# lRomul/sensorium

Hardware: AMD Instinct MI355X
Metric: training clips/sec/GPU (DwiseNeuro fwd+bwd, B=32 T=32 36x64) at 1/2/4/8 GPUs (higher is better)
Workload: dtype bf16

## Files before the change

sensorium_amd/csrc/dwn_api.hip:

```cpp
#include "dwn_internal.h"
#include "dwn_kernels.h"
#include <string.h>
#include <math.h>

static thread_local char g_err[512] = "";
#ifndef DWN_EVAL_CHAIN
#define DWN_EVAL_CHAIN 1
#endif

extern "C" size_t dwn_dw_spatial_rc_blob_bytes(int E, int Cin);
extern "C" int dwn_dw_spatial_rc_supported(int dtype, int Cin, int E, int ks, int stride, int Hin, int Win);
extern "C" int dwn_dw_spatial_rc_prep(const float* w_pw, const float* w_dws, const float* bn1_coef, int E, int Cin, void* blob,
                                      int device, void* stream);
extern "C" int dwn_dw_spatial_fwd_rc(const dwn_dw_spatial_rc_fwd_args* a, int device, void* stream);
bool dw_spatial_bwd_rc_supported(const DwSpatialBwd& a, int dtype);
bool dw_spatial_fwd_rc_walk_supported(const DwSpatialFwd& a, int dtype);

int dwn_set_error(int code, const char* msg) {
    snprintf(g_err, sizeof(g_err), "dwn error %d: %s", code, msg ? msg : "");
    return code;
}

#define TRY(x) do { int rc__ = (x); if (rc__ != 0) return rc__; } while (0)

// ... 110 lines not shown
}

int bn_finalize(const double* stats, int stat_c, double count, const dwn_bn& bn, int C, int training, float momentum,
                float eps, hipStream_t s) {
    if (training) return k_bn_finalize_train(fin_job(stats, stat_c, count, bn, C), BnFinJob{}, momentum, eps, s);
    return k_bn_finalize_eval(bn.gamma, bn.beta, bn.running_mean, bn.running_var, eps, bn.coef, C, s);
}

GemmNN nn_base(const LoadDesc& a, int a_kind, const void* b, i64 ldb, void* c, i64 ldc, int M, int N, int K, int groups) {
    GemmNN g; memset(&g, 0, sizeof(g));
    g.a = a; g.a_kind = a_kind; g.b = b; g.ldb = ldb; g.c = c; g.ldc = ldc; g.M = M; g.N = N; g.K = K;
    g.groups = groups; g.epi = EPI_STORE;
    return g;
}
GemmTN tn_base(const LoadDesc& p, int pk, const LoadDesc& q, int qk, int M, int R, int Cc, float* dw, i64 lddw, int groups) {
    GemmTN g; memset(&g, 0, sizeof(g));
    g.p = p; g.p_kind = pk; g.q = q; g.q_kind = qk; g.M = M; g.R = R; g.Cc = Cc; g.dw = dw; g.lddw = lddw;
    g.groups = groups; g.nsplit = 0;
    return g;
}

struct BlockWs {
    void *wpw, *wpwl;
    float *wdws, *wdwt;
    double *st1, *st2, *st3, *st4, *stsc;
    long long* pooled;
    float *abc1, *abc2, *abc3, *abc4, *abcsc, *ident3;
    float *dgp, *dhp, *dps;
    void* bp; float* r3; float* gacc;
    float* tacc;
    void* wgated;
    void* rcblob;
    double* gram;
    float* pb;
    char* zero_beg; char* zero_end;
    size_t bytes;
};
#ifndef PWL_GATED_MIN_ROWS
#define PWL_GATED_MIN_ROWS 8192
#endif
static bool pwl_gated_weights(const dwn_block_args& a) {
    const int bk = a.dtype == DWN_BF16 ? 64 : 32;
    return ((a.T * a.Hout * a.Wout) % 128) == 0 && a.Cmid > bk && (a.dtype != DWN_BF16 || a.T * a.Hout * a.Wout >= PWL_GATED_MIN_ROWS);
}
static bool pwl_bwd_per_sample(const dwn_block_args& a) {
#ifdef DWN_DETERMINISTIC
    return true;
#endif
    if (a.pwl_bwd == 2) return false;
    if (a.pwl_bwd == 1) return true;
    const double pb = 4.0 * a.B * a.Cout * a.Cmid * sizeof(float);
    const double pass = (double)a.B * a.T * a.Hout * a.Wout * a.Cmid * tsize(a.dtype);
    return pb <= pass;
}
static bool block_y1_free(const dwn_block_args& a) {
    if (!a.training || a.dtype != DWN_BF16 || a.y1_mode == 1) return false;
    DwSpatialFwd f; memset(&f, 0, sizeof(f));
    f.planes = a.B * a.T; f.Hin = a.Hin; f.Win = a.Win; f.Hout = a.Hout; f.Wout = a.Wout; f.C = a.Cmid; f.stride = a.stride; f.ks = a.ks;
    f.in.ld = a.Cmid; f.a0_ld = a.Cin; f.Cin = a.Cin;
    if (!dw_spatial_fwd_rc_walk_supported(f, a.dtype)) return false;
    DwSpatialBwd d; memset(&d, 0, sizeof(d));
    d.planes = a.B * a.T; d.Hin = a.Hin; d.Win = a.Win; d.Hout = a.Hout; d.Wout = a.Wout; d.C = a.Cmid; d.stride = a.stride; d.ks = a.ks;
    d.dy.ld = a.Cmid; d.y1.ld = a.Cmid; d.a0_ld = a.Cin; d.Cin = a.Cin;
    if (!dw_spatial_bwd_rc_supported(d, a.dtype)) return false;
    return a.y1_mode == 2 || a.Cin == 64;
}
static bool block_fwd_rc(const dwn_block_args& a) {
    return !a.training && dwn_dw_spatial_rc_supported(a.dtype, a.Cin, a.Cmid, a.ks, a.stride, a.Hin, a.Win) != 0;
}
static size_t pw_fold_floats(int Cin) { return (size_t)Cin * Cin + Cin; }
BlockWs carve_block(const dwn_block_args& a, int backward, void* base, size_t cap) {
    BlockWs w; memset(&w, 0, sizeof(w));
    Carver c(base, cap);
    const size_t ts = tsize(a.dtype);
    w.wpw = c.take<char>((size_t)a.Cmid * a.Cin * ts);
    w.wpwl = c.take<char>((size_t)a.Cout * a.Cmid * ts);
    w.wdws = c.take<float>((size_t)a.ks * a.ks * a.Cmid);
    w.wdwt = c.take<float>((size_t)a.kt * a.Cmid);
    if (!backward && pwl_gated_weights(a)) w.wgated = c.take<char>((size_t)a.B * a.Cout * a.Cmid * ts);
    if (!backward && block_fwd_rc(a)) w.rcblob = c.take<char>(dwn_dw_spatial_rc_blob_bytes(a.Cmid, a.Cin));
    c.take<char>(0);
    size_t z0 = (c.off + 255) & ~(size_t)255;
    w.st1 = c.take<double>(nstat(a.Cmid));
    w.st2 = c.take<double>(nstat(a.Cmid));
    w.st3 = c.take<double>(nstat(a.Cmid));
    w.st4 = c.take<double>(nstat(a.Cout));
    w.stsc = c.take<double>(nstat(backward ? a.Cout : a.Cin));
    w.pooled = c.take<long long>((size_t)a.B * a.Cmid);
    if (!backward && block_y1_free(a)) w.gram = c.take<double>((size_t)(a.Cin + 8) * a.Cin);
    size_t z1 = c.off;
    if (backward) {
        w.abc1 = c.take<float>(3 * (size_t)a.Cmid);
        w.abc2 = c.take<float>(3 * (size_t)a.Cmid);
        w.abc3 = c.take<float>(3 * (size_t)a.Cmid);
        w.abc4 = c.take<float>(3 * (size_t)a.Cout);
        w.abcsc = c.take<float>(3 * (size_t)a.Cout);
        w.ident3 = c.take<float>(3 * (size_t)a.Cmid);
        w.dgp = c.take<float>((size_t)a.B * a.Cmid);
        w.dhp = c.take<float>((size_t)a.B * a.se_r);
        w.dps = c.take<float>((size_t)a.B * a.Cmid);
        w.bp = c.take<char>((size_t)a.Cin * (a.Cmid + a.Cin) * ts);
        w.gacc = c.take<float>(pw_fold_floats(a.Cin));
        w.r3 = w.gacc + (size_t)a.Cin * a.Cin;
        w.tacc = c.take<float>(pw_wgrad_tacc_floats(a.Cmid, a.Cin));
        if (pwl_bwd_per_sample(a)) w.pb = c.take<float>((size_t)a.B * a.Cout * a.Cmid);
    }
    w.bytes = c.off + 256;
    if (base) { w.zero_beg = (char*)base + z0; w.zero_end = (char*)base + z1; }
    return w;
}

static inline int f32_split_of(int policy, bool eval_forward) {
    return policy == DWN_F32_SPLIT3 ? 1 : policy == DWN_F32_NATIVE ? 0 : (eval_forward ? 1 : 0);
}

ResGeom geom_of(const dwn_block_args& a) {
    ResGeom gm;
    gm.BT = a.B * a.T; gm.T = a.T; gm.Hin = a.Hin; gm.Win = a.Win; gm.Hout = a.Hout; gm.Wout = a.Wout;
    gm.Cin = a.Cin; gm.Cout = a.Cout; gm.hsrc = a.hsrc; gm.wsrc = a.wsrc; gm.hinv = a.hinv; gm.winv = a.winv;
    return gm;
}

int check_block(const dwn_block_args& a) {
// ... 72 lines not shown
int dwn_dw_spatial_fwd_rc_supported(const dwn_dw_spatial_fwd_args* a, int dtype) { return dw_spatial_fwd_rc_walk_supported(*a, dtype) ? 1 : 0; }
int dwn_dw_temporal_fwd(const dwn_dw_temporal_fwd_args* a, int dtype, int device, void* stream) {
    ENTER(device);
    if (a->kt != 3 && a->kt != 5) return dwn_set_error(-4, "dw_temporal: only temporal_kernel 3 or 5 is built");
    return launch_dw_temporal_fwd(*a, dtype, (hipStream_t)stream);
}
int dwn_dw_temporal_bwd(const dwn_dw_temporal_bwd_args* a, int dtype, int device, void* stream) {
    ENTER(device);
    if (a->kt != 3 && a->kt != 5) return dwn_set_error(-4, "dw_temporal: only temporal_kernel 3 or 5 is built");
    return launch_dw_temporal_bwd(*a, dtype, (hipStream_t)stream);
}
int dwn_dw_temporal_wide_fwd(const dwn_dw_temporal_fwd_args* a, int dtype, int device, void* stream) {
    g_err[0] = 0;
    if (int rc = dw_temporal_wide_check(a->kt, a->C, LD_PLAIN)) return rc;
    ENTER(device);
    return launch_dw_temporal_wide_fwd(*a, dtype, (hipStream_t)stream);
}
int dwn_dw_temporal_wide_bwd(const dwn_dw_temporal_bwd_args* a, int dtype, int device, void* stream) {
    g_err[0] = 0;
    if (int rc = dw_temporal_wide_check(a->kt, a->C, a->dy_kind)) return rc;
    ENTER(device);
    return launch_dw_temporal_wide_bwd(*a, dtype, (hipStream_t)stream);
}
int dwn_bn_finalize(const double* stats, int stat_c, double count, const dwn_bn* bn, int C, int training,
                    float momentum, float eps, int device, void* stream) {
    ENTER(device);
    return bn_finalize(stats, stat_c, count, *bn, C, training, momentum, eps, (hipStream_t)stream);
}
int dwn_bn_bwd_finalize(const double* stats, double count, const dwn_bn* bn, float* abc, int C, int device,
                        void* stream) {
    ENTER(device);
    return k_bn_bwd_finalize(bwd_job(stats, count, *bn, abc, C, false), BnBwdJob{}, (hipStream_t)stream);
}
size_t dwn_conv_pw_bn_stats_workspace_bytes(int Cin) { return (size_t)(Cin + 8) * Cin * sizeof(double) + 256; }
int dwn_conv_pw_bn_stats(const void* a0, long long a0_ld, long long M, const float* w_pw, int E, int Cin, const dwn_bn* bn,
                         float momentum, float eps, double* sc_stats, void* ws, size_t ws_bytes, int dtype, int device, void* stream) {
    ENTER(device);
    hipStream_t s = (hipStream_t)stream;
    if (!a0 || !w_pw || !bn || !bn->coef || !ws) return dwn_set_error(-1, "conv_pw_bn_stats: null pointer");
    if (Cin % 8 || E <= 0 || M <= 0 || M >= (1ll << 31)) return dwn_set_error(-2, "conv_pw_bn_stats: Cin % 8 == 0, 0 < M < 2^31");
    if (ws_bytes < dwn_conv_pw_bn_stats_workspace_bytes(Cin)) return dwn_set_error(-6, "conv_pw_bn_stats: workspace too small");
    double* gram = reinterpret_cast<double*>(((size_t)ws + 255) & ~(size_t)255);
    TRY(k_zero(gram, (size_t)(Cin + 8) * Cin * sizeof(double), s));
    LoadDesc cat = ld_plain(a0, a0_ld);
    cat.cat_c1 = Cin; cat.cat_c2 = 0;
    GemmTN g = tn_base(cat, LD_CAT1, ld_plain(a0, a0_ld), LD_PLAIN, (int)M, Cin + 8, Cin, reinterpret_cast<float*>(gram), Cin, 1);
    g.dw_f64 = 1;
    TRY(launch_gemm_tn(g, dtype, s));
    return k_bn1_gram_finalize(gram, w_pw, E, Cin, (double)M, bn->gamma, bn->beta, bn->running_mean, bn->running_var,
                               bn->num_batches_tracked, momentum, eps, bn->coef, sc_stats, dtype, s);
}
int dwn_pack_weight(const float* src, void* dst, int groups, int R, int C, int transpose, int Rd, int Cd, int dtype,
                    int device, void* stream) {
    ENTER(device);
    return k_pack_weight(src, dst, groups, R, C, transpose, Rd, Cd, dtype, (hipStream_t)stream);
}

size_t dwn_stem_workspace_bytes(const dwn_stem_args* a) {
    return ((size_t)DWN_NREP * stem_moment_count() * sizeof(double) + 256 +
            (size_t)DWN_NREP * a->C0 * stem_acc_stride() * sizeof(double) + 1024);
}
int dwn_stem_forward(const dwn_stem_args* a, int device, void* stream) {
    ENTER(device);
    hipStream_t s = (hipStream_t)stream;
    if (a->C0 % 8) return dwn_set_error(-2, "stem: C0 must be a multiple of 8");
    if (a->pe_t && (i64)a->T * a->H * a->W != a->S) return dwn_set_error(-2, "stem: T*H*W != S");
    Carver c(a->ws, a->ws_bytes);
    double* mom = c.take<double>((size_t)DWN_NREP * stem_moment_count());
    if (!c.ok()) return dwn_set_error(-6, "stem: workspace too small");
    const i64 M = (i64)a->B * a->S;
    if (a->training == DWN_BN_TRAIN) {
        if (!a->xmom) return dwn_set_error(-1, "stem_forward: xmom buffer required in training mode");
        TRY(k_zero(mom, (size_t)DWN_NREP * stem_moment_count() * sizeof(double), s));
        TRY(k_stem_xmom(a->x, a->B, a->Cin, a->S, mom, s));
        TRY(k_stem_bn_finalize(mom, (double)M, a->w, a->bn.gamma, a->bn.beta, a->bn.running_mean, a->bn.running_var,
// ... 91 lines not shown
            ok = ok && pa.bneval(a.bn1, a.Cmid, a.eps) && pa.bneval(a.bn2, a.Cmid, a.eps) && pa.bneval(a.bn3, a.Cmid, a.eps);
            ok = ok && pa.bneval(a.bn4, a.Cout, a.eps) && pa.bneval(a.bnsc, a.Cout, a.eps);
        }
        if (!ok) return dwn_set_error(-2, "block_forward: workspace arena must be 16-byte aligned");
        TRY(k_prep(pa, dt, s));
    }

    const void* a0 = a.x;
    if (!a.x_has_pe) {
        if (!a.a0) return dwn_set_error(-2, "block_forward: a0 buffer required when x_has_pe == 0");
        TRY(k_ew_apply(ld_pe(a.x, a.Cin, a.pe_t, a.pe_h, a.pe_w, a.T, a.Hin, a.Win), LD_PE, a.a0, a.Cin, Min, a.Cin, dt, s));
        a0 = a.a0;
    }
    LoadDesc xin = ld_plain(a0, a.Cin);
    const bool identity_sc = a.stride == 1 && a.Hin == a.Hout && a.Win == a.Wout;
    const bool y1_free = tr && block_y1_free(a);
    bool eval_chain = false;
    if (DWN_EVAL_CHAIN && !tr && dt == DWN_BF16) {
        DwSpatialFwd f; memset(&f, 0, sizeof(f));
        f.planes = a.B * a.T; f.Hin = a.Hin; f.Win = a.Win; f.Hout = a.Hout; f.Wout = a.Wout; f.C = a.Cmid; f.stride = a.stride; f.ks = a.ks;
        f.in.ld = a.Cmid; f.a0_ld = a.Cin; f.Cin = a.Cin;
        eval_chain = dw_spatial_fwd_rc_walk_supported(f, dt);
    }
    if (eval_chain) {
        DwSpatialFwd d; memset(&d, 0, sizeof(d));
        d.in = ld_bnact(nullptr, a.Cmid, a.bn1.coef, a.Cmid, 1, nullptr, 0, 1);
        d.a0 = a0; d.a0_ld = a.Cin; d.w1 = w.wpw; d.Cin = a.Cin;
        d.w = w.wdws; d.out = a.y2; d.planes = a.B * a.T; d.Hin = a.Hin; d.Win = a.Win; d.Hout = a.Hout;
        d.Wout = a.Wout; d.C = a.Cmid; d.stride = a.stride; d.ks = a.ks; d.stats = nullptr;
        PROF(DWN_FAM_DWS_FWD, launch_dw_spatial_fwd(d, dt, s));
    } else if (y1_free) {
        LoadDesc cat = ld_plain(a0, a.Cin);
        cat.cat_c1 = a.Cin; cat.cat_c2 = 0;
        if (bs) {
        GemmTN g = tn_base(cat, LD_CAT1, ld_plain(a0, a.Cin), LD_PLAIN, (int)Min, a.Cin + 8, a.Cin, reinterpret_cast<float*>(w.gram), a.Cin, 1);
        g.dw_f64 = 1;
        PROF(DWN_FAM_PW_FWD, launch_gemm_tn(g, dt, s));
        PROF(DWN_FAM_PW_FWD, k_bn1_gram_finalize(w.gram, a.w_pw, a.Cmid, a.Cin, (double)Min, a.bn1.gamma, a.bn1.beta, a.bn1.running_mean,
                                                 a.bn1.running_var, a.bn1.num_batches_tracked, a.momentum, a.eps, a.bn1.coef,
                                                 identity_sc ? w.stsc : nullptr, dt, s));
        }
        DwSpatialFwd d; memset(&d, 0, sizeof(d));
        d.in = ld_bnact(nullptr, a.Cmid, a.bn1.coef, a.Cmid, 1, nullptr, 0, 1);
        d.a0 = a0; d.a0_ld = a.Cin; d.w1 = w.wpw; d.Cin = a.Cin;
        d.w = w.wdws; d.out = a.y2; d.planes = a.B * a.T; d.Hin = a.Hin; d.Win = a.Win; d.Hout = a.Hout;
        d.Wout = a.Wout; d.C = a.Cmid; d.stride = a.stride; d.ks = a.ks; d.stats = w.st2;
        PROF(DWN_FAM_DWS_FWD, launch_dw_spatial_fwd(d, dt, s));
    } else if (block_fwd_rc(a)) {
        TRY(dwn_dw_spatial_rc_prep(a.w_pw, w.wdws, a.bn1.coef, a.Cmid, a.Cin, w.rcblob, device, stream));
        dwn_dw_spatial_rc_fwd_args r; memset(&r, 0, sizeof(r));
        r.a0 = a0; r.a0_ld = a.Cin; r.blob = w.rcblob; r.out = a.y2; r.planes = a.B * a.T; r.Hin = a.Hin; r.Win = a.Win;
        r.Hout = a.Hout; r.Wout = a.Wout; r.Cin = a.Cin; r.E = a.Cmid; r.stride = a.stride; r.stats = nullptr;
        r.rows_band = 0; r.round_y1 = 1;
        PROF(DWN_FAM_DWS_FWD, dwn_dw_spatial_fwd_rc(&r, device, stream));
    } else {
    {
        GemmNN g = nn_base(xin, LD_PLAIN, w.wpw, a.Cin, a.y1, a.Cmid, (int)Min, a.Cmid, a.Cin, 1);
        g.f32_split = f32_split_of(a.f32_products, !tr);
        g.stats = tr ? w.st1 : nullptr; g.stat_nchan = a.Cmid;
        PROF(DWN_FAM_PW_FWD, launch_gemm_nn(g, dt, s));
    }
    if (bs) TRY(bn_finalize(w.st1, a.Cmid, (double)Min, a.bn1, a.Cmid, 1, a.momentum, a.eps, s));
    {
        DwSpatialFwd d; memset(&d, 0, sizeof(d));
        d.in = ld_bnact(a.y1, a.Cmid, a.bn1.coef, a.Cmid, 1, nullptr, 0, 1);
        d.w = w.wdws; d.out = a.y2; d.planes = a.B * a.T; d.Hin = a.Hin; d.Win = a.Win; d.Hout = a.Hout;
        d.Wout = a.Wout; d.C = a.Cmid; d.stride = a.stride; d.ks = a.ks; d.stats = tr ? w.st2 : nullptr;
// ... 584 lines not shown
```

sensorium_amd/csrc/dwn_elementwise.hip:

```cpp
#include "dwn_internal.h"
#include "dwn_kernels.h"
#include "dwn_launch.h"

#define NCV 8
#define DISPATCH_T(dtype, CALL_BF, CALL_F) do { if ((dtype) == DWN_BF16) { CALL_BF; } else { CALL_F; } } while (0)

#define SLICE_SETUP(Cval)                                   \
    constexpr int KC = TT<T>::KC;                           \
    const int tid = threadIdx.x;                            \
    const int cv = tid % NCV, pl = tid / NCV;               \
    const int c0 = blockIdx.y * NCV * KC;                   \
    const int chan = c0 + cv * KC;                          \
    const bool chan_ok = chan < (Cval);                     \
    (void)pl; (void)chan_ok;

template <int KC>
__device__ __forceinline__ void slice_stats_flush(float* lstat, const float* s0, const float* s1, int cv,
                                                 int c0, int C, double* stats, int rep) {
    static_assert(NCV == 8, "wave pre-reduction below assumes 8 channel vectors per slice");
    const int tid = threadIdx.x;
    DET_WAVES_BEGIN
#pragma unroll
    for (int i = 0; i < KC; ++i) {
        float a = s0[i], b = s1[i];
// ... 168 lines not shown
    }
#pragma unroll
    for (int o = 32; o > 0; o >>= 1) { quad += __shfl_xor(quad, o); lin += __shfl_xor(lin, o); }
    if (lane != 0) return;
    const double mean = lin * inv_n;
    double var = quad * inv_n - mean * mean;
    if (var < 0) var = 0;
    const float invstd = (float)(1.0 / sqrt(var + (double)eps));
    const float scale = gamma[e] * invstd;
    coef[e] = scale;
    coef[E + e] = beta[e] - (float)mean * scale;
    coef[2 * E + e] = (float)mean;
    coef[3 * E + e] = invstd;
    if (running_mean) {
        const double unbiased = count > 1 ? var * count / (count - 1) : var;
        running_mean[e] = (1.f - momentum) * running_mean[e] + momentum * (float)mean;
        running_var[e] = (1.f - momentum) * running_var[e] + momentum * (float)unbiased;
    }
}
int k_bn1_gram_finalize(const double* gram, const float* w1, int E, int Cin, double count, const float* gamma, const float* beta,
                        float* rm, float* rv, long long* nbt, float momentum, float eps, float* coef, double* sc_stats, int dtype,
                        hipStream_t s) {
    if (Cin > 512 || Cin % 4) return dwn_set_error(-2, "bn1_gram_finalize: Cin must be a multiple of 4, at most 512");
    if (dtype == DWN_BF16)
        hipLaunchKernelGGL(bn1_gram_finalize_kernel<bf16_t>, dim3((E + 3) / 4), dim3(256), 0, s, gram, w1, E, Cin, count, gamma, beta,
                           rm, rv, nbt, momentum, eps, coef, sc_stats);
    else
        hipLaunchKernelGGL(bn1_gram_finalize_kernel<float>, dim3((E + 3) / 4), dim3(256), 0, s, gram, w1, E, Cin, count, gamma, beta,
                           rm, rv, nbt, momentum, eps, coef, sc_stats);
    DWN_CHECK_LAUNCH();
    return 0;
}

template <typename T, int KIND>
__global__ __launch_bounds__(256) void ew_apply_kernel(LoadDesc d, T* out, i64 ldo, i64 rows, int C) {
    SLICE_SETUP(C)
    if (!chan_ok) return;
    for (i64 row = (i64)blockIdx.x * 32 + pl; row < rows; row += (i64)gridDim.x * 32) {
        float v[KC];
        load_op<KIND, T>(d, row, chan, v);
        st_vec<T>(out + row * ldo + chan, v);
    }
}

template <typename T>
static int ew_apply_t(const LoadDesc& d, int kind, void* out, i64 ldo, i64 rows, int C, hipStream_t s) {
    dim3 grid = slice_grid(rows, C, TT<T>::KC);
    T* o = reinterpret_cast<T*>(out);
    switch (kind) {
        case LD_PLAIN: hipLaunchKernelGGL((ew_apply_kernel<T, LD_PLAIN>), grid, dim3(256), 0, s, d, o, ldo, rows, C); break;
        case LD_PE: hipLaunchKernelGGL((ew_apply_kernel<T, LD_PE>), grid, dim3(256), 0, s, d, o, ldo, rows, C); break;
        case LD_BNACT: hipLaunchKernelGGL((ew_apply_kernel<T, LD_BNACT>), grid, dim3(256), 0, s, d, o, ldo, rows, C); break;
        case LD_AFFINE2: hipLaunchKernelGGL((ew_apply_kernel<T, LD_AFFINE2>), grid, dim3(256), 0, s, d, o, ldo, rows, C); break;
        case LD_DY3: hipLaunchKernelGGL((ew_apply_kernel<T, LD_DY3>), grid, dim3(256), 0, s, d, o, ldo, rows, C); break;
        case LD_GATE: hipLaunchKernelGGL((ew_apply_kernel<T, LD_GATE>), grid, dim3(256), 0, s, d, o, ldo, rows, C); break;
        default: return dwn_set_error(-3, "ew_apply: bad loader kind");
    }
    DWN_CHECK_LAUNCH();
    return 0;
}
int k_ew_apply(const LoadDesc& d, int kind, void* out, i64 ldo, i64 rows, int C, int dtype, hipStream_t s) {
    return dtype == DWN_BF16 ? ew_apply_t<bf16_t>(d, kind, out, ldo, rows, C, s)
                             : ew_apply_t<float>(d, kind, out, ldo, rows, C, s);
}

constexpr int STEM_MAXCIN = 8;
// ... 2435 lines not shown
```

sensorium_amd/csrc/dwn_gemm.hip:

```cpp
#include "dwn_internal.h"
#include "dwn_launch.h"
#include <type_traits>
int k_zero(void* p, size_t nbytes, hipStream_t s);

#ifndef NN_DMA_NST
#define NN_DMA_NST 3
#endif
#ifndef NN_F32_X3
#define NN_F32_X3 1
#endif

typedef __attribute__((ext_vector_type(8))) short bf16x8_t;
typedef __attribute__((ext_vector_type(4))) short s16x4_t;
typedef __attribute__((ext_vector_type(4))) float f32x4_t;

template <typename T> struct Mma;
template <> struct Mma<bf16_t> {
    static __device__ __forceinline__ void run(const uint4& a, const uint4& b, f32x4_t& acc) {
        acc = __builtin_amdgcn_mfma_f32_16x16x32_bf16(__builtin_bit_cast(bf16x8_t, a),
                                                      __builtin_bit_cast(bf16x8_t, b), acc, 0, 0, 0);
    }
};
template <> struct Mma<float> {
    static __device__ __forceinline__ void run(const uint4& a, const uint4& b, f32x4_t& acc) {
// ... 1000 lines not shown
    }
    dim3 grid(((g.R + 127) / 128) * ((g.Cc + 127) / 128), g.nsplit, g.groups);
    hipLaunchKernelGGL((gemm_tn_kernel<T, PLD, QLD>), grid, dim3(256), 0, s, g);
    DWN_CHECK_LAUNCH();
    return 0;
}

template <typename T>
static int launch_tn_d(const GemmTN& g, hipStream_t s) {
    const int Rl = g.R_load > 0 ? g.R_load : g.R;
    if (Rl % TT<T>::KC != 0 || g.Cc % TT<T>::KC != 0)
        return dwn_set_error(-2, "gemm_tn: R and Cc must be multiples of the 16-byte vector");
    const int pk = g.p_kind, qk = g.q_kind;
    if (pk == LD_AFFINE2 && qk == LD_PE) return launch_tn_t<T, LD_AFFINE2, LD_PE>(g, s);
    if (pk == LD_PLAIN && qk == LD_BNACT) return launch_tn_t<T, LD_PLAIN, LD_BNACT>(g, s);
    if (pk == LD_PLAIN && qk == LD_GATE) return launch_tn_t<T, LD_PLAIN, LD_GATE>(g, s);
    if (pk == LD_PLAIN && qk == LD_PLAIN) return launch_tn_t<T, LD_PLAIN, LD_PLAIN>(g, s);
    if (pk == LD_AFFINE2 && qk == LD_PLAIN) return launch_tn_t<T, LD_AFFINE2, LD_PLAIN>(g, s);
    if (pk == LD_CAT1 && qk == LD_PLAIN) {
        if (g.p.cat_c1 <= 0 || g.p.cat_c2 < 0 || g.p.cat_c1 % TT<T>::KC || g.p.cat_c2 % TT<T>::KC || g.groups != 1 ||
            g.R < g.p.cat_c1 + g.p.cat_c2 || (g.p.cat_c2 > 0 && !g.p.q))
            return dwn_set_error(-2, "gemm_tn: LD_CAT1 needs groups == 1, segment widths in 16-byte vectors and R >= cat_c1 + cat_c2");
        return launch_tn_t<T, LD_CAT1, LD_PLAIN>(g, s);
    }
    return dwn_set_error(-3, "gemm_tn: unsupported loader combination");
}

int launch_gemm_tn(const GemmTN& g_in, int dtype, hipStream_t s) {
    if (g_in.M <= 0 || g_in.R <= 0 || g_in.Cc <= 0) return 0;
    const GemmTN& g = g_in;
    return dtype == DWN_BF16 ? launch_tn_d<bf16_t>(g, s) : launch_tn_d<float>(g, s);
}

static __device__ __forceinline__ unsigned pwb_pack2(float a, float b) { return pk_bf16(a, b); }
namespace pwb {
constexpr int CIN = 64, BM = 128;
constexpr int RS = 160;
template <int NKC> struct Cfg {
    static constexpr int E = NKC * 64, KCAT = E + CIN;
    static constexpr int WRS = KCAT * 2 + 16;
    static constexpr int SW_BYTES = CIN * WRS, SD_BYTES = BM * RS, SX_BYTES = BM * RS;
    static constexpr int MAP_INTS = 512;
    static constexpr int LDS_BYTES = SW_BYTES + 2 * SD_BYTES + 2 * SX_BYTES + 7 * CIN * 4 + MAP_INTS * 4;
};
}
struct PwbGather { const int* hinv; const int* winv; int Hin, Win, Hout, Wout; };
template <int NKC>
__global__ __launch_bounds__(512) __attribute__((amdgpu_waves_per_eu(2, 2))) void pw_bwd_fused_kernel(const bf16_t* __restrict__ dh1, const bf16_t* __restrict__ a0,
                                                       const bf16_t* __restrict__ bp, const float* __restrict__ r3,
                                                       bf16_t* __restrict__ da0, float* __restrict__ tacc, int M,
                                                       const bf16_t* __restrict__ res, const float* __restrict__ res_coef, int res_n,
                                                       const PwbGather gq) {
    using namespace pwb;
    constexpr int E = Cfg<NKC>::E, KCAT = Cfg<NKC>::KCAT, WRS = Cfg<NKC>::WRS;
    constexpr int SW_BYTES = Cfg<NKC>::SW_BYTES, SD_BYTES = Cfg<NKC>::SD_BYTES, SX_BYTES = Cfg<NKC>::SX_BYTES;
    extern __shared__ __attribute__((aligned(16))) unsigned char pwb_smem[];
    unsigned char* const smem = pwb_smem;
    unsigned char* sW = smem;
    unsigned char* sD = smem + SW_BYTES;
    unsigned char* sX = sD + 2 * SD_BYTES;
    float* sR3 = reinterpret_cast<float*>(sX + 2 * SX_BYTES);
    const int tid = threadIdx.x, wave = tid >> 6, lane = tid & 63;
    const int lr = lane & 15, lg = lane >> 4;
    const int wm = wave & 3, wn = wave >> 2;
    if (tid < CIN) sR3[tid] = r3[tid];
    const bool gather = res && gq.hinv;
// ... 238 lines not shown
```

sensorium_amd/csrc/dwn_internal.h:

```cpp
#pragma once
#include "dwn_common.h"

enum { EPI_STORE = DWN_EPI_STORE, EPI_READOUT = DWN_EPI_READOUT, EPI_DG = DWN_EPI_DG, EPI_STORE_CAT = DWN_EPI_STORE_CAT, EPI_DH3 = DWN_EPI_DH3,
       EPI_READOUT_LB = 100 };
typedef dwn_gemm_nn_args GemmNN;
typedef dwn_gemm_tn_args GemmTN;
typedef dwn_dw_spatial_fwd_args DwSpatialFwd;
typedef dwn_dw_spatial_bwd_args DwSpatialBwd;
typedef dwn_dw_temporal_fwd_args DwTemporalFwd;
typedef dwn_dw_temporal_bwd_args DwTemporalBwd;

int launch_gemm_nn(const GemmNN& g, int dtype, hipStream_t s);
int launch_gemm_tn(const GemmTN& g, int dtype, hipStream_t s);
bool gemm_nn_xl_eligible(const GemmNN& g, int dtype);
int launch_gemm_nn_xl(const GemmNN& g, hipStream_t s);
bool gemm_nn_kd_eligible(const GemmNN& g, int dtype);
int launch_gemm_nn_kd(const GemmNN& g, hipStream_t s);
int launch_dw_spatial_fwd(const DwSpatialFwd& a, int dtype, hipStream_t s);
int launch_dw_spatial_bwd(const DwSpatialBwd& a, int dtype, hipStream_t s);
int launch_dw_temporal_fwd(const DwTemporalFwd& a, int dtype, hipStream_t s);
int launch_dw_temporal_bwd(const DwTemporalBwd& a, int dtype, hipStream_t s);
int dw_temporal_wide_check(int kt, int C, int dy_kind);
int launch_dw_temporal_wide_fwd(const DwTemporalFwd& a, int dtype, hipStream_t s);
int launch_dw_temporal_wide_bwd(const DwTemporalBwd& a, int dtype, hipStream_t s);
bool pw_bwd_fused_supported(int dtype, long long M, int E, int Cin);
int launch_pw_bwd_fused(const void* dh1, const void* a0, const void* bp, const float* r3, void* da0, float* tacc,
                        long long M, int E, int Cin, int dtype, const void* res, const float* res_coef, int res_n,
                        const int* hinv, const int* winv, int Hin, int Win, int Hout, int Wout, hipStream_t s);
```

sensorium_amd/csrc/dwn_kernels.h:

```cpp
#pragma once
#include "dwn_internal.h"

struct ResGeom {
    int BT, T, Hin, Win, Hout, Wout, Cin, Cout;
    const int* hsrc; const int* wsrc;
    const int* hinv; const int* winv;
};

typedef dwn_tensor_entry TensorListEntry;

struct BnFinJob {
    const double* stats; int stat_c; double count; const float* gamma; const float* beta;
    float* running_mean; float* running_var; long long* nbt; float* coef; int C; int nblocks;
};
struct BnBwdJob { const double* stats; double count; const float* coef; float* dgamma; float* dbeta; float* abc; int C; int nblocks; int frozen; };
int k_bn_finalize_train(BnFinJob j0, BnFinJob j1, float momentum, float eps, hipStream_t s);
int k_bn_bwd_finalize(BnBwdJob j0, BnBwdJob j1, hipStream_t s);
int k_bn_finalize_eval(const float* gamma, const float* beta, const float* rm, const float* rv, float eps,
                       float* coef, int C, hipStream_t s);
int k_bn1_gram_finalize(const double* gram, const float* w1, int E, int Cin, double count, const float* gamma, const float* beta,
                        float* rm, float* rv, long long* nbt, float momentum, float eps, float* coef, double* sc_stats, int dtype,
                        hipStream_t s);
int k_ew_apply(const LoadDesc& d, int kind, void* out, i64 ldo, i64 rows, int C, int dtype, hipStream_t s);
int k_stem_xmom(const float* x, int B, int Cin, i64 S, double* mom, hipStream_t s);
int k_stem_bn_finalize(const double* mom, double count, const float* w, const float* gamma, const float* beta, float* rm,
                       float* rv, long long* nbt, float momentum, float eps, float* coef, double* xmom, int C0, int Cin,
                       hipStream_t s);
int k_stem_out(const float* x, const float* w, const float* coef, const float* pe_t, const float* pe_h, const float* pe_w,
               int Tn, int H, int W, int B, int Cin, i64 S, int C0, void* out, int dtype, hipStream_t s);
int k_stem_bwd_acc(const void* dout, const float* x, const double* xmom, double count, int B, int Cin, i64 S, int C0,
                   double* acc, int dtype, hipStream_t s);
int k_stem_bwd_finalize(const double* acc, const double* xmom, const float* w, const float* coef, double count, float* dgamma,
                        float* dbeta, float* dw, int C0, int Cin, hipStream_t s);
int k_stem_bwd_finalize_frozen(const double* acc, const float* w, const float* coef, float* dgamma, float* dbeta, float* dw,
                               int C0, int Cin, hipStream_t s);
int k_stem_input_grad(const void* dout, const float* w, const float* coef, int B, int Cin, i64 S, int C0, float* dx, int dtype,
                      hipStream_t s);
int k_stem_bwd_finalize_dx(const double* acc, const double* xmom, const float* w, const float* coef, double count, float* qx,
                           int C0, int Cin, hipStream_t s);
int k_stem_input_grad_train(const void* dout, const float* w, const float* coef, const float* x, const float* qx, int B, int Cin,
                            i64 S, int C0, float* dx, int dtype, hipStream_t s);
int stem_moment_count();
int stem_acc_stride();
int k_shortcut_stats(const LoadDesc& xin, const ResGeom& gm, double* stats, int dtype, hipStream_t s);
int k_residual_fwd(const LoadDesc& xin, const void* y4, const float* coef4, const float* coefsc, const float* dscale,
                   const ResGeom& gm, const float* ope_t, const float* ope_h, const float* ope_w, void* out, int dtype,
                   hipStream_t s);
int k_residual_bwd_reduce(const LoadDesc& xin, const void* y4, const void* dout, const float* coef4,
                          const float* coefsc, const float* dscale, const ResGeom& gm, double* stats4,
                          double* statssc, int dtype, hipStream_t s);
int k_residual_bwd_dy4(const void* y4, const void* dout, const float* abc4, const float* dscale, const ResGeom& gm,
                       void* dy4, int dtype, hipStream_t s);
int k_residual_bwd_dx(const LoadDesc& xin, const void* da0, const void* dout, const float* abcsc, const ResGeom& gm,
                      void* dx, int dtype, hipStream_t s);
int k_se_pool(const LoadDesc& z3, int B, int C, int rows_per_sample, long long* pooled, void* z3out, int dtype, hipStream_t s);
// ... 112 lines not shown
```

Measured before the change: 1452.

## Compute BN1 Gram statistics with dedicated MFMA partial-slab kernel and fused fold-finalize

```diff
diff --git a/sensorium_amd/csrc/dwn_api.hip b/sensorium_amd/csrc/dwn_api.hip
--- a/sensorium_amd/csrc/dwn_api.hip
+++ b/sensorium_amd/csrc/dwn_api.hip
@@ -166,6 +166,7 @@
     void* wgated;
     void* rcblob;
     double* gram;
+    unsigned* gcnt; double* gslabs; double* gqpart;
     float* pb;
     char* zero_beg; char* zero_end;
     size_t bytes;
@@ -201,6 +202,9 @@
 }
 static bool block_fwd_rc(const dwn_block_args& a) {
     return !a.training && dwn_dw_spatial_rc_supported(a.dtype, a.Cin, a.Cmid, a.ks, a.stride, a.Hin, a.Win) != 0;
+}
+static bool gram_fold_route(int dtype, int Cin, int E, i64 a0_ld, const void* a0) {
+    return gram_partials_supported(dtype, Cin, a0_ld, a0) && E <= 128 * GRAM_MAX_CHUNKS;
 }
 static size_t pw_fold_floats(int Cin) { return (size_t)Cin * Cin + Cin; }
 BlockWs carve_block(const dwn_block_args& a, int backward, void* base, size_t cap) {
@@ -221,8 +225,14 @@
     w.st4 = c.take<double>(nstat(a.Cout));
     w.stsc = c.take<double>(nstat(backward ? a.Cout : a.Cin));
     w.pooled = c.take<long long>((size_t)a.B * a.Cmid);
-    if (!backward && block_y1_free(a)) w.gram = c.take<double>((size_t)(a.Cin + 8) * a.Cin);
+    const bool gfold = !backward && block_y1_free(a) && gram_fold_route(a.dtype, a.Cin, a.Cmid, a.Cin, nullptr);
+    if (gfold) w.gcnt = c.take<unsigned>(64);
+    else if (!backward && block_y1_free(a)) w.gram = c.take<double>((size_t)(a.Cin + 8) * a.Cin);
     size_t z1 = c.off;
+    if (gfold) {
+        w.gslabs = c.take<double>((size_t)GRAM_MAX_SLABS * GRAM_SLAB);
+        w.gqpart = c.take<double>(bn1_gram_fold_qpart_doubles(a.Cmid));
+    }
     if (backward) {
         w.abc1 = c.take<float>(3 * (size_t)a.Cmid);
         w.abc2 = c.take<float>(3 * (size_t)a.Cmid);
@@ -361,7 +371,12 @@
     ENTER(device);
     return k_bn_bwd_finalize(bwd_job(stats, count, *bn, abc, C, false), BnBwdJob{}, (hipStream_t)stream);
 }
-size_t dwn_conv_pw_bn_stats_workspace_bytes(int Cin) { return (size_t)(Cin + 8) * Cin * sizeof(double) + 256; }
+size_t dwn_conv_pw_bn_stats_workspace_bytes(int Cin) {
+    size_t n = (size_t)(Cin + 8) * Cin * sizeof(double) + 256;
+    if (Cin == 64 || Cin == 128)
+        n += 256 + (size_t)GRAM_MAX_SLABS * GRAM_SLAB * sizeof(double) + 256 + bn1_gram_fold_qpart_doubles(128 * GRAM_MAX_CHUNKS) * sizeof(double);
+    return n;
+}
 int dwn_conv_pw_bn_stats(const void* a0, long long a0_ld, long long M, const float* w_pw, int E, int Cin, const dwn_bn* bn,
                          float momentum, float eps, double* sc_stats, void* ws, size_t ws_bytes, int dtype, int device, void* stream) {
     ENTER(device);
@@ -370,6 +385,16 @@
     if (Cin % 8 || E <= 0 || M <= 0 || M >= (1ll << 31)) return dwn_set_error(-2, "conv_pw_bn_stats: Cin % 8 == 0, 0 < M < 2^31");
     if (ws_bytes < dwn_conv_pw_bn_stats_workspace_bytes(Cin)) return dwn_set_error(-6, "conv_pw_bn_stats: workspace too small");
     double* gram = reinterpret_cast<double*>(((size_t)ws + 255) & ~(size_t)255);
+    if (gram_fold_route(dtype, Cin, E, a0_ld, a0)) {
+        unsigned* cnt = reinterpret_cast<unsigned*>(gram + (size_t)(Cin + 8) * Cin);
+        double* slabs = reinterpret_cast<double*>(cnt + 64);
+        double* qpart = slabs + (size_t)GRAM_MAX_SLABS * GRAM_SLAB;
+        int nslice = 0;
+        TRY(k_zero(cnt, 256, s));
+        TRY(launch_gram_partials(a0, a0_ld, M, Cin, slabs, &nslice, s));
+        return k_bn1_gram_fold(slabs, nslice, w_pw, E, Cin, (double)M, bn->gamma, bn->beta, bn->running_mean, bn->running_var,
+                               bn->num_batches_tracked, momentum, eps, bn->coef, sc_stats, qpart, cnt, s);
+    }
     TRY(k_zero(gram, (size_t)(Cin + 8) * Cin * sizeof(double), s));
     LoadDesc cat = ld_plain(a0, a0_ld);
     cat.cat_c1 = Cin; cat.cat_c2 = 0;
@@ -527,7 +552,14 @@
     } else if (y1_free) {
         LoadDesc cat = ld_plain(a0, a.Cin);
         cat.cat_c1 = a.Cin; cat.cat_c2 = 0;
-        if (bs) {
+        if (bs && w.gcnt && ((size_t)a0 & 15) == 0) {
+        int nslice = 0;
+        PROF(DWN_FAM_PW_FWD, launch_gram_partials(a0, a.Cin, Min, a.Cin, w.gslabs, &nslice, s));
+        PROF(DWN_FAM_PW_FWD, k_bn1_gram_fold(w.gslabs, nslice, a.w_pw, a.Cmid, a.Cin, (double)Min, a.bn1.gamma, a.bn1.beta,
+                                             a.bn1.running_mean, a.bn1.running_var, a.bn1.num_batches_tracked, a.momentum, a.eps,
+                                             a.bn1.coef, identity_sc ? w.stsc : nullptr, w.gqpart, w.gcnt, s));
+        } else if (bs) {
+        if (!w.gram) return dwn_set_error(-2, "block_forward: the block input must be 16-byte aligned");
         GemmTN g = tn_base(cat, LD_CAT1, ld_plain(a0, a.Cin), LD_PLAIN, (int)Min, a.Cin + 8, a.Cin, reinterpret_cast<float*>(w.gram), a.Cin, 1);
         g.dw_f64 = 1;
         PROF(DWN_FAM_PW_FWD, launch_gemm_tn(g, dt, s));
diff --git a/sensorium_amd/csrc/dwn_elementwise.hip b/sensorium_amd/csrc/dwn_elementwise.hip
--- a/sensorium_amd/csrc/dwn_elementwise.hip
+++ b/sensorium_amd/csrc/dwn_elementwise.hip
@@ -224,6 +224,126 @@
     return 0;
 }
 
+template <typename T>
+__global__ __launch_bounds__(256) void bn1_gram_finalize_fold_kernel(const double* slabs, int nslice, const float* __restrict__ w1,
+                                                                     int E, int Cin, double count, const float* gamma, const float* beta,
+                                                                     float* running_mean, float* running_var, long long* nbt,
+                                                                     float momentum, float eps, float* coef, double* sc_stats,
+                                                                     double2* qpart, unsigned* cnt) {
+    __shared__ double part[4][4][64];
+    __shared__ double grow[4][128];
+    __shared__ double wsum[4][4], ssum[4];
+    __shared__ int last;
+    const int t = threadIdx.x, lane = t & 63, wv = t >> 6;
+    const int RPW = Cin >> 5, i0 = blockIdx.x * RPW, ch = blockIdx.y;
+    if (blockIdx.x == 0 && ch == 0 && t == 0 && nbt) *nbt += 1;
+    const int col = t & (Cin - 1), grp = t / Cin, ngrp = 256 / Cin;
+    const int per = (nslice + ngrp - 1) / ngrp;
+    const int sbeg = grp * per, send = sbeg + per < nslice ? sbeg + per : nslice;
+    double* partf = &part[0][0][0];
+    for (int r = 0; r < RPW; ++r) {
+        const int i = i0 + r;
+        int tile = 0, scol = col;
+        double f = 1.0;
+        bool on = true;
+        if (Cin == 128) {
+            if (i < 64) { if (col >= 64) { tile = 1; scol = col - 64; f = 2.0; } }
+            else if (col < 64) on = false;
+            else { tile = 2; scol = col - 64; }
+        }
+        double a = 0.0;
+        if (on) {
+            const double* p = slabs + ((i64)tile * nslice + sbeg) * GRAM_SLAB + (i & 63) * 64 + scol;
+#pragma unroll 8
+            for (int sl = sbeg; sl < send; ++sl, p += GRAM_SLAB) a += *p;
+        }
+        partf[(grp * RPW + r) * Cin + col] = a * f;
+        const int dtile = (Cin == 128 && i >= 64) ? 2 : 0;
+        double sv = t < nslice ? slabs[((i64)dtile * nslice + t) * GRAM_SLAB + 64 * 64 + (i & 63)] : 0.0;
+#pragma unroll
+        for (int o = 32; o > 0; o >>= 1) sv += __shfl_xor(sv, o);
+        if (lane == 0) wsum[r][wv] = sv;
+    }
+    __syncthreads();
+    for (int idx = t; idx < RPW * Cin; idx += 256) {
+        const int r = idx / Cin, c = idx - r * Cin;
+        double g = 0.0;
+        for (int k = 0; k < ngrp; ++k) g += partf[(k * RPW + r) * Cin + c];
+        grow[r][c] = g;
+    }
+    if (t < RPW) ssum[t] = ((wsum[t][0] + wsum[t][1]) + wsum[t][2]) + wsum[t][3];
+    __syncthreads();
+    if (sc_stats && ch == 0 && t < RPW) {
+        sc_stats[i0 + t] = ssum[t];
+        sc_stats[Cin + i0 + t] = grow[t][i0 + t];
+    }
+    const int e = ch * 128 + t;
+    if (t < 128 && e < E) {
+        const float* we = w1 + (i64)e * Cin;
+        double dot[4] = {0.0, 0.0, 0.0, 0.0};
+        for (int j = 0; j < Cin; j += 4) {
+            const double wj[4] = {(double)round_t<T>(we[j]), (double)round_t<T>(we[j + 1]), (double)round_t<T>(we[j + 2]),
+                                  (double)round_t<T>(we[j + 3])};
+#pragma unroll
+            for (int r = 0; r < 4; ++r)
+                if (r < RPW) dot[r] += ((grow[r][j] * wj[0] + grow[r][j + 1] * wj[1]) + grow[r][j + 2] * wj[2]) + grow[r][j + 3] * wj[3];
+        }
+        double quad = 0.0, lin = 0.0;
+#pragma unroll
+        for (int r = 0; r < 4; ++r)
+            if (r < RPW) {
+                const double wi = (double)round_t<T>(we[i0 + r]);
+                quad += wi * dot[r];
+                lin += wi * ssum[r];
+            }
+        qpart[((i64)ch * 32 + blockIdx.x) * 128 + t] = make_double2(quad, lin);
+    }
+    asm volatile("s_waitcnt vmcnt(0)" ::: "memory");
+    __syncthreads();
+    if (t == 0) {
+        __builtin_amdgcn_fence(__ATOMIC_RELEASE, "agent");
+        asm volatile("s_waitcnt vmcnt(0)" ::: "memory");
+        const unsigned old = __hip_atomic_fetch_add(cnt + ch, 1u, __ATOMIC_RELAXED, __HIP_MEMORY_SCOPE_AGENT);
+        last = old == gridDim.x - 1;
+        if (last) {
+            __builtin_amdgcn_fence(__ATOMIC_ACQUIRE, "agent");
+            asm volatile("s_waitcnt vmcnt(0)" ::: "memory");
+        }
+    }
+    __syncthreads();
+    if (!last || t >= 128 || e >= E) return;
+    double quad = 0.0, lin = 0.0;
+    const double2* qp = qpart + (i64)ch * 32 * 128 + t;
+#pragma unroll 8
+    for (int k = 0; k < 32; ++k) { const double2 v = qp[k * 128]; quad += v.x; lin += v.y; }
+    const double inv_n = 1.0 / count;
+    const double mean = lin * inv_n;
+    double var = quad * inv_n - mean * mean;
+    if (var < 0) var = 0;
+    const float invstd = (float)(1.0 / sqrt(var + (double)eps));
+    const float scale = gamma[e] * invstd;
+    coef[e] = scale;
+    coef[E + e] = beta[e] - (float)mean * scale;
+    coef[2 * E + e] = (float)mean;
+    coef[3 * E + e] = invstd;
+    if (running_mean) {
+        const double unbiased = count > 1 ? var * count / (count - 1) : var;
+        running_mean[e] = (1.f - momentum) * running_mean[e] + momentum * (float)mean;
+        running_var[e] = (1.f - momentum) * running_var[e] + momentum * (float)unbiased;
+    }
+}
+size_t bn1_gram_fold_qpart_doubles(int E) { return (size_t)((E + 127) / 128) * 32 * 128 * 2; }
+int k_bn1_gram_fold(const double* slabs, int nslice, const float* w1, int E, int Cin, double count, const float* gamma,
+                    const float* beta, float* rm, float* rv, long long* nbt, float momentum, float eps, float* coef, double* sc_stats,
+                    double* qpart, unsigned* cnt, hipStream_t s) {
+    if ((Cin != 64 && Cin != 128) || nslice < 1 || nslice > 256 || E < 1 || (E + 127) / 128 > GRAM_MAX_CHUNKS)
+        return dwn_set_error(-2, "bn1_gram_fold: Cin 64 or 128, at most 256 slabs per tile and 128 * GRAM_MAX_CHUNKS channels");
+    hipLaunchKernelGGL(bn1_gram_finalize_fold_kernel<bf16_t>, dim3(32, (E + 127) / 128), dim3(256), 0, s, slabs, nslice, w1, E, Cin, count,
+                       gamma, beta, rm, rv, nbt, momentum, eps, coef, sc_stats, reinterpret_cast<double2*>(qpart), cnt);
+    DWN_CHECK_LAUNCH();
+    return 0;
+}
+
 template <typename T, int KIND>
 __global__ __launch_bounds__(256) void ew_apply_kernel(LoadDesc d, T* out, i64 ldo, i64 rows, int C) {
     SLICE_SETUP(C)
diff --git a/sensorium_amd/csrc/dwn_gemm.hip b/sensorium_amd/csrc/dwn_gemm.hip
--- a/sensorium_amd/csrc/dwn_gemm.hip
+++ b/sensorium_amd/csrc/dwn_gemm.hip
@@ -1056,6 +1056,128 @@
     return dtype == DWN_BF16 ? launch_tn_d<bf16_t>(g, s) : launch_tn_d<float>(g, s);
 }
 
+constexpr int GRAM_STEP = 256;
+constexpr int GRAM_RUN = 2;
+template <int NC>
+static __device__ __forceinline__ void gram_tile(const bf16_t* a0, i64 ld, i64 mbeg, i64 mend, int lc0, int ac, int bc,
+                                                 double* slab, unsigned char* smem) {
+    constexpr int RS = NC * 2 + 32;
+    constexpr int CPR = NC / 8, NCH = GRAM_STEP * CPR / 512, RPI = 512 / CPR;
+    const int tid = threadIdx.x, wave = tid >> 6, lane = tid & 63, lr = lane & 15, lg = lane >> 4;
+    const int chq = tid % CPR, row0 = tid / CPR;
+    const bf16_t* src = a0 + lc0 + chq * 8;
+    uint4 v[NCH];
+    auto load_rows = [&](i64 mb) {
+#pragma unroll
+        for (int i = 0; i < NCH; ++i) {
+            const i64 m = mb + row0 + RPI * i;
+            v[i] = *reinterpret_cast<const uint4*>(src + (m < mend ? m : mbeg) * ld);
+        }
+    };
+    auto store_rows = [&](i64 mb) {
+#pragma unroll
+        for (int i = 0; i < NCH; ++i) {
+            const int r = row0 + RPI * i;
+            *reinterpret_cast<uint4*>(smem + r * RS + chq * 16) = (mb + r < mend) ? v[i] : make_uint4(0, 0, 0, 0);
+        }
+    };
+    const int ti = wave >> 1, tj = (wave & 1) * 2;
+    const int q = lr >> 2, p = lr & 3;
+    const int acol = (ac - lc0 + ti * 16 + 4 * p) * 2, bcol = (bc - lc0 + tj * 16 + 4 * p) * 2;
+    const bf16x8_t ones = {0x3F80, 0x3F80, 0x3F80, 0x3F80, 0x3F80, 0x3F80, 0x3F80, 0x3F80};
+    f32x4_t acc[2], accs[2];
+    double dacc[2][4], dsum[2];
+#pragma unroll
+    for (int j = 0; j < 2; ++j) {
+        acc[j] = accs[j] = f32x4_t{0.f, 0.f, 0.f, 0.f};
+        dsum[j] = 0.0;
+#pragma unroll
+        for (int r = 0; r < 4; ++r) dacc[j][r] = 0.0;
+    }
+    auto frag = [&](int rb, int colb) {
+        auto lo = __builtin_amdgcn_ds_read_tr16_b64_v4i16((__attribute__((address_space(3))) s16x4_t*)(smem + rb * RS + colb));
+        auto hi = __builtin_amdgcn_ds_read_tr16_b64_v4i16((__attribute__((address_space(3))) s16x4_t*)(smem + (rb + 4) * RS + colb));
+        return bf16x8_t{lo[0], lo[1], lo[2], lo[3], hi[0], hi[1], hi[2], hi[3]};
+    };
+    load_rows(mbeg);
+    store_rows(mbeg);
+    __syncthreads();
+    int run = 0;
+    for (i64 mb = mbeg; mb < mend; mb += GRAM_STEP) {
+        const bool has_next = mb + GRAM_STEP < mend;
+        if (has_next) load_rows(mb + GRAM_STEP);
+#pragma unroll
+        for (int kb = 0; kb < GRAM_STEP / 32; ++kb) {
+            const int rb = kb * 32 + 8 * lg + q;
+            const bf16x8_t af = frag(rb, acol);
+#pragma unroll
+            for (int j = 0; j < 2; ++j) {
+                const bf16x8_t bfr = frag(rb, bcol + j * 32);
+                acc[j] = __builtin_amdgcn_mfma_f32_16x16x32_bf16(af, bfr, acc[j], 0, 0, 0);
+                if (ti == 0) accs[j] = __builtin_amdgcn_mfma_f32_16x16x32_bf16(ones, bfr, accs[j], 0, 0, 0);
+            }
+        }
+        if (++run == GRAM_RUN || !has_next) {
+            run = 0;
+#pragma unroll
+            for (int j = 0; j < 2; ++j) {
+#pragma unroll
+                for (int r = 0; r < 4; ++r) dacc[j][r] += (double)acc[j][r];
+                dsum[j] += (double)accs[j][0];
+                acc[j] = accs[j] = f32x4_t{0.f, 0.f, 0.f, 0.f};
+            }
+        }
+        __syncthreads();
+        if (has_next) {
+            store_rows(mb + GRAM_STEP);
+            __syncthreads();
+        }
+    }
+#pragma unroll
+    for (int j = 0; j < 2; ++j) {
+#pragma unroll
+        for (int r = 0; r < 4; ++r) slab[(ti * 16 + lg * 4 + r) * 64 + (tj + j) * 16 + lr] = dacc[j][r];
+        if (ti == 0 && lg == 0) slab[64 * 64 + (tj + j) * 16 + lr] = dsum[j];
+    }
+}
+__global__ __launch_bounds__(512) void bn1_gram_partial_kernel(const bf16_t* a0, i64 ld, i64 M, int Cin, int nslice, i64 rows,
+                                                               double* slabs) {
+    extern __shared__ __attribute__((aligned(16))) unsigned char gram_smem[];
+    int quad = 0, slice = blockIdx.x;
+    if (Cin == 128) {
+        const int g = blockIdx.x / 24, r = blockIdx.x % 24;
+        quad = r >> 3;
+        slice = g * 8 + (r & 7);
+    }
+    if (slice >= nslice) return;
+    const i64 mbeg = (i64)slice * rows;
+    const i64 mend = mbeg + rows < M ? mbeg + rows : M;
+    double* slab = slabs + ((i64)quad * nslice + slice) * GRAM_SLAB;
+    if (quad == 1) gram_tile<128>(a0, ld, mbeg, mend, 0, 0, 64, slab, gram_smem);
+    else gram_tile<64>(a0, ld, mbeg, mend, quad * 32, quad * 32, quad * 32, slab, gram_smem);
+}
+
+bool gram_partials_supported(int dtype, int Cin, i64 a0_ld, const void* a0) {
+    return dtype == DWN_BF16 && (Cin == 64 || Cin == 128) && a0_ld >= Cin && a0_ld % 8 == 0 && ((size_t)a0 & 15) == 0;
+}
+int launch_gram_partials(const void* a0, i64 a0_ld, i64 M, int Cin, double* slabs, int* nslice, hipStream_t s) {
+    if (M <= 0 || !gram_partials_supported(DWN_BF16, Cin, a0_ld, a0)) return dwn_set_error(-2, "gram_partials: bf16, Cin 64 or 128, 16-byte rows");
+    const int maxs = Cin == 64 ? GRAM_MAX_SLABS : GRAM_MAX_SLABS / 3 / 8 * 8;
+    i64 n = (M + GRAM_STEP - 1) / GRAM_STEP;
+    if (n > maxs) n = maxs;
+    i64 rows = (M + n - 1) / n;
+    rows = (rows + GRAM_STEP - 1) / GRAM_STEP * GRAM_STEP;
+    n = (M + rows - 1) / rows;
+    *nslice = (int)n;
+    const size_t lds = (size_t)GRAM_STEP * (Cin * 2 + 32);
+    if (lds_opt_in(bn1_gram_partial_kernel, lds) != hipSuccess) (void)hipGetLastError();
+    const unsigned grid = Cin == 64 ? (unsigned)n : (unsigned)((n + 7) / 8 * 24);
+    hipLaunchKernelGGL(bn1_gram_partial_kernel, dim3(grid), dim3(512), lds, s, reinterpret_cast<const bf16_t*>(a0), a0_ld, M, Cin,
+                       (int)n, rows, slabs);
+    DWN_CHECK_LAUNCH();
+    return 0;
+}
+
 static __device__ __forceinline__ unsigned pwb_pack2(float a, float b) { return pk_bf16(a, b); }
 namespace pwb {
 constexpr int CIN = 64, BM = 128;
diff --git a/sensorium_amd/csrc/dwn_internal.h b/sensorium_amd/csrc/dwn_internal.h
--- a/sensorium_amd/csrc/dwn_internal.h
+++ b/sensorium_amd/csrc/dwn_internal.h
@@ -12,6 +12,11 @@
 
 int launch_gemm_nn(const GemmNN& g, int dtype, hipStream_t s);
 int launch_gemm_tn(const GemmTN& g, int dtype, hipStream_t s);
+constexpr int GRAM_SLAB = 65 * 64;
+constexpr int GRAM_MAX_SLABS = 256;
+constexpr int GRAM_MAX_CHUNKS = 32;
+bool gram_partials_supported(int dtype, int Cin, i64 a0_ld, const void* a0);
+int launch_gram_partials(const void* a0, i64 a0_ld, i64 M, int Cin, double* slabs, int* nslice, hipStream_t s);
 bool gemm_nn_xl_eligible(const GemmNN& g, int dtype);
 int launch_gemm_nn_xl(const GemmNN& g, hipStream_t s);
 bool gemm_nn_kd_eligible(const GemmNN& g, int dtype);
diff --git a/sensorium_amd/csrc/dwn_kernels.h b/sensorium_amd/csrc/dwn_kernels.h
--- a/sensorium_amd/csrc/dwn_kernels.h
+++ b/sensorium_amd/csrc/dwn_kernels.h
@@ -21,6 +21,10 @@
 int k_bn1_gram_finalize(const double* gram, const float* w1, int E, int Cin, double count, const float* gamma, const float* beta,
                         float* rm, float* rv, long long* nbt, float momentum, float eps, float* coef, double* sc_stats, int dtype,
                         hipStream_t s);
+size_t bn1_gram_fold_qpart_doubles(int E);
+int k_bn1_gram_fold(const double* slabs, int nslice, const float* w1, int E, int Cin, double count, const float* gamma,
+                    const float* beta, float* rm, float* rv, long long* nbt, float momentum, float eps, float* coef, double* sc_stats,
+                    double* qpart, unsigned* cnt, hipStream_t s);
 int k_ew_apply(const LoadDesc& d, int kind, void* out, i64 ldo, i64 rows, int C, int dtype, hipStream_t s);
 int k_stem_xmom(const float* x, int B, int Cin, i64 S, double* mom, hipStream_t s);
 int k_stem_bn_finalize(const double* mom, double count, const float* w, const float* gamma, const float* beta, float* rm,
```

Result: no change. 1458, median of 6 (+0.4%).
